# mayabechlerspeicher/Graph-Neural-Additive-Networks---GNAN

Hardware: AMD Instinct MI355X
Metric: edges aggregated/sec, TensorGNAN forward (higher is better)
Workload: dtype f32

## Files before the change

graph-neural-additive-networks---gnan_amd/_lib.py:

```python
from __future__ import annotations

import ctypes as C
import os
from typing import Optional

import torch

_HERE = os.path.dirname(os.path.abspath(__file__))
LIB_PATH = os.environ.get("GNAN_HIP_LIB") or os.path.join(_HERE, "libgnan_hip.so")
ABI_VERSION = 51
ERR_BAD_ARG, ERR_UNSUPPORTED, ERR_HIP, ERR_WORKSPACE = -1, -2, -3, -4

GNAN_F32, GNAN_BF16 = 0, 1
FMLP_AUTO, FMLP_LANE, FMLP_MFMA, FMLP_PWL = 0, 1, 2, 3
MAX_CODES = 256


class GnanHipError(RuntimeError):
    pass


class FmlpArgs(C.Structure):
    _fields_ = [
        ("x", C.c_void_p), ("n", C.c_int64), ("x_stride", C.c_int64),
# ... 130 lines not shown
        ("s_total", C.c_void_p), ("weight_by_col", C.c_int32), ("minus_rest", C.c_int32),
        ("reduce_cr", C.c_int32), ("scatter_out", C.c_int32), ("Y", C.c_void_p), ("y_stride", C.c_int64),
        ("long_threshold", C.c_int64), ("long_rows", C.c_void_p), ("long_slice_ptr", C.c_void_p),
        ("n_long", C.c_int32), ("n_slices", C.c_int32), ("slice_edges", C.c_int32),
        ("workspace", C.c_void_p), ("workspace_bytes", C.c_size_t),
        ("s_by_code", C.c_int32), ("nnz", C.c_int64), ("packed_index", C.c_int32),
        ("hot_lo", C.c_int64), ("hot_rows", C.c_int32), ("shell_out", C.c_void_p),
        ("cls_index", C.c_void_p), ("cls_slice_start", C.c_void_p), ("cls_slice_row", C.c_void_p), ("cls_slot_slice", C.c_void_p),
        ("cls_n_slots", C.c_int32),
        ("short_lmax", C.c_int32), ("short_row", C.c_void_p), ("short_pair", C.c_void_p),
        ("self_sum", C.c_void_p), ("self_parts", C.c_int32),
        ("seg_index", C.c_void_p), ("seg_start", C.c_void_p), ("seg_row", C.c_void_p), ("cls_seg_ptr", C.c_void_p),
        ("seg_mask", C.c_void_p), ("seg_q_lo", C.c_int64), ("seg_q_hi", C.c_int64), ("n_seg", C.c_int32),
        ("seg_max_per_class", C.c_int32),
        ("hub_index", C.c_void_p), ("hub_seg_start", C.c_void_p), ("hub_seg_row", C.c_void_p), ("hub_seg_slot", C.c_void_p),
        ("hub_row_slot_ptr", C.c_void_p), ("hub_cls_seg_ptr", C.c_void_p), ("hub_q_lo", C.c_int64), ("n_hub", C.c_int32),
        ("n_hub_seg", C.c_int32), ("hub_seg_max_per_class", C.c_int32),
        ("stream_index", C.c_void_p), ("stream_cls_pair_ptr", C.c_void_p), ("stream_cls_chunk_ptr", C.c_void_p),
        ("stream_chunk_first_seg", C.c_void_p), ("stream_seg_slot", C.c_void_p), ("stream_row_slot_ptr", C.c_void_p),
        ("stream_q_lo", C.c_int64), ("stream_q_hi", C.c_int64), ("stream_chunk", C.c_int32), ("stream_code", C.c_int32),
        ("n_stream_seg", C.c_int32), ("stream_max_chunks_per_class", C.c_int32),
        ("stream_row_seg", C.c_void_p),
        ("q_hub", C.c_int64),
    ]


SHORT_LMAX = 8
SPMM_KERNEL_NONE, SPMM_KERNEL_ROWS, SPMM_KERNEL_HOT = 0, 1, 2


class SpmmLaunchInfo(C.Structure):
    _fields_ = [
        ("vec", C.c_int32), ("lpr", C.c_int32), ("smalld", C.c_int32), ("dense", C.c_int32), ("kernel", C.c_int32),
        ("classed", C.c_int32), ("n_slice_blocks", C.c_int32), ("n_tile_blocks", C.c_int32), ("n_tiles", C.c_int32),
        ("row_q0", C.c_int64), ("short_tile", C.c_int32 * (SHORT_LMAX + 1)),
        ("n_seg_blocks", C.c_int32), ("n_segs", C.c_int32), ("n_hub_seg_blocks", C.c_int32), ("n_hub_segs", C.c_int32),
        ("n_stream_blocks", C.c_int32), ("n_stream_segs", C.c_int32),
    ]

    def as_dict(self) -> dict:
        d = {name: getattr(self, name) for name, _ in self._fields_}
        d["short_tile"] = list(self.short_tile)
        return d


class ClassedPlanArgs(C.Structure):
    _fields_ = [
        ("rowptr", C.c_void_p), ("rowptr_is64", C.c_int32), ("col", C.c_void_p), ("code", C.c_void_p), ("row_ids", C.c_void_p),
        ("long_rows", C.c_void_p), ("n_long", C.c_int32), ("slice_edges", C.c_int32),
        ("workspace", C.c_void_p), ("workspace_bytes", C.c_size_t), ("totals", C.c_void_p),
        ("index", C.c_void_p), ("slice_start", C.c_void_p), ("slice_row", C.c_void_p), ("slice_ptr", C.c_void_p),
        ("slot_slice", C.c_void_p), ("n_slots", C.c_int64),
    ]


class SortedCsrArgs(C.Structure):
    _fields_ = [
        ("n_rows", C.c_int64), ("nnz", C.c_int64), ("rowptr", C.c_void_p), ("rowptr_is64", C.c_int32), ("col", C.c_void_p),
        ("code", C.c_void_p), ("cnt", C.c_void_p), ("D", C.c_int32), ("pack_shift", C.c_int32), ("order", C.c_void_p),
        ("rowptr_s", C.c_void_p), ("col_s", C.c_void_p), ("code_s", C.c_void_p), ("colp_s", C.c_void_p), ("cnt_s", C.c_void_p),
        ("workspace", C.c_void_p), ("workspace_bytes", C.c_size_t),
    ]


class CsrTransposeArgs(C.Structure):
    _fields_ = [
# ... 561 lines not shown
```

graph-neural-additive-networks---gnan_amd/aggregate.py:

```python
from __future__ import annotations

import functools
from dataclasses import dataclass
from typing import NamedTuple, Optional

import torch

from . import _lib
from . import functional as Fn
from .functional import StackedMLP
from .graph import LONG_ROW_THRESHOLD, HopGraph

DENSE_SLICE_MAX_ROWS = 16384
DENSE_SLICE_MIN_COLS = 512
WEIGHT_TABLE_MAX_BYTES = 1 << 30
NARROW_DS_MAX_WIDTH = 32


def _spmm_args(g: HopGraph, S, lut, use_cnt, s_total, out, row_ids, per_row_lut, weight_by_col=False,
               minus_rest=False, plan=None, workspace=None, reduce_cr=0, scatter_out=False,
               s_by_code=False, packed=False, hot_rows=0) -> _lib.SpmmArgs:
    D, Cw = lut.shape[-2], lut.shape[-1]
    packed = bool(packed and PACKED_INDEX and g.colp is not None and D <= 4 and Cw == 1 and not weight_by_col
                  and not minus_rest and not s_by_code)
# ... 24 lines not shown


def _hot_head_in_lds(g: HopGraph, head: int) -> bool:
    return g.hot_head_share(head) >= HOT_LDS_MIN_SHARE


FUSABLE_READOUT = (1, 2, 4)
DEGREE_SCHEDULE_MIN_WIDTH = 8
DEGREE_SORTED_COPY_MIN_ROWS = 1 << 16
WIDE_INDEX_LOADS = True
PACKED_INDEX = True
NARROW_SORTED_MIN_NNZ = 1 << 23
NARROW_SORTED_WALK = True
HOT_COLUMN_ROWS = True
HOT_ROWS_IN_LDS = True
HOT_LDS_FLOATS = 16384
HOT_LDS_MIN_SHARE = 0.25
DEGREE_SORTED_COPY = True
XCD_CLASSED_HUBS = True
CLASSED_MIN_ROW_BYTES = 128
CLASSED_MIN_NNZ = 1 << 24
SHORT_ROW_TILES = True
SHORT_ROW_LMAX = 4
CLASSED_ROWS = True
CLASSED_ROWS_MIN_NNZ = 1 << 24
CLASSED_ROWS_MIN_PAIRS = 33
BLOCKED_HUBS = True
BLOCKED_HUBS_MIN_NNZ = 1 << 24
BLOCKED_HUB_BLOCK_BYTES = 4 << 20
BLOCKED_HUB_BLOCKS = 4
BLOCKED_HUB_SEG_PAIRS = 256
PAIR_STREAM = True
PAIR_STREAM_MIN_NNZ = 1 << 24
PAIR_STREAM_MIN_PAIRS = 5
PAIR_STREAM_BLOCKS = 2
PAIR_STREAM_CHUNK_PAIRS = 32
HUB_STREAM = True
HUB_STREAM_MIN_NNZ = 1 << 24
HUB_STREAM_BLOCKS = 4
HUB_STREAM_CHUNK_PAIRS = 32
PAIR_STREAM_COMBINE_ROWS = 256
PAIR_STREAM_COMBINE_CAP = 4096


def append_hot_rows(S: torch.Tensor, hot: torch.Tensor, group: int = 1, room: Optional[torch.Tensor] = None) -> torch.Tensor:
    W = S.shape[1]
# ... 84 lines not shown
    else:
        by_col_table = per_row and weight_by_col and not use_cnt
        g, row_ids, plan, scatter = _wide_walk(g, row_ids, S.shape[1], by_col_table or (not per_row and not weight_by_col))
        short = scatter == 2 and SHORT_ROW_TILES and not per_row and not weight_by_col
    if (XCD_CLASSED_HUBS and plan is not None and not g.is_dense and S.shape[1] * S.element_size() >= CLASSED_MIN_ROW_BYTES
            and g.nnz >= CLASSED_MIN_NNZ and not weight_by_col and not minus_rest and not s_by_code and not g._cnt_by_col
            and n_hot == 0):
        classed = g.classed_hub_plan(row_ids if scatter != 2 else None)
        if classed is not None:
            plan = classed
    if from_counts:
        lut = lut_of_counts(g.cnt).detach().float().contiguous()
        per_row = True
    a = _spmm_args(g, S, lut, use_cnt, s_total, out, row_ids, per_row, weight_by_col, minus_rest, plan,
                   reduce_cr=reduce_cr, scatter_out=scatter, s_by_code=s_by_code, packed=True, hot_rows=n_hot)
    if short and a.packed_index:
        runs = g.short_row_runs(SHORT_ROW_LMAX)
        a.short_lmax, a.short_row, a.short_pair = runs.lmax, runs.row_ptr, runs.pair_ptr
    if self_sum is not None:
        _lib.require_device(self_sum)
        if self_sum.dtype != torch.float32 or self_sum.dim() != 2 or self_sum.shape[1] != n_out or not self_sum.is_contiguous():
            raise ValueError("self_sum must be a contiguous float32 [parts, n_rows] tensor")
        a.self_sum, a.self_parts = _lib.ptr(self_sum), int(self_sum.shape[0])
        if (scatter == 2 and a.packed_index and a.short_lmax > 0 and reduce_cr == 1 and s_total is not None
                and S.dtype == torch.float32 and (plan is None or plan.threshold == LONG_ROW_THRESHOLD)):
            W, lo, rows, hubs, both = S.shape[1], SHORT_ROW_LMAX + 1, None, None, None
            block_rows = max(1, BLOCKED_HUB_BLOCK_BYTES // (W * 4)) if W else 0
            if (HUB_STREAM and PAIR_STREAM and HUB_STREAM_CHUNK_PAIRS == PAIR_STREAM_CHUNK_PAIRS and g.nnz >= HUB_STREAM_MIN_NNZ
                    and 32 < W <= 256 and plan is not None and plan.n_long > 0):
                both = g.pair_stream_plan(max(PAIR_STREAM_MIN_PAIRS, lo), block_rows, PAIR_STREAM_BLOCKS, HUB_STREAM_CHUNK_PAIRS, None,
                                          HUB_STREAM_BLOCKS)
            if both is not None:
                both.bind(a)
            else:
                if PAIR_STREAM and g.nnz >= PAIR_STREAM_MIN_NNZ and 32 < W <= 256:
                    rows = g.pair_stream_plan(max(PAIR_STREAM_MIN_PAIRS, lo), block_rows, PAIR_STREAM_BLOCKS, PAIR_STREAM_CHUNK_PAIRS)
                if rows is None and CLASSED_ROWS and g.nnz >= CLASSED_ROWS_MIN_NNZ:
                    rows = g.classed_row_plan(max(CLASSED_ROWS_MIN_PAIRS, lo))
                if BLOCKED_HUBS and g.nnz >= BLOCKED_HUBS_MIN_NNZ and plan is not None and plan.n_long > 0:
                    hubs = g.blocked_hub_plan(block_rows, BLOCKED_HUB_BLOCKS, BLOCKED_HUB_SEG_PAIRS)
                for wide in (rows, hubs):
                    if wide is not None:
                        wide.bind(a)
    need = _lib.lib().gnan_spmm_fwd_workspace_bytes(a)
    ws = None
    if need:
# ... 677 lines not shown
```

graph-neural-additive-networks---gnan_amd/csrc/spmm.hip:

```cpp
#include "spmm_common.hpp"

namespace {

template <int VEC>
__device__ __forceinline__ Vec<VEC> hot_gather(const Params& p, const float* hot, int c) {
  const int64_t r = static_cast<int64_t>(c) - p.hot_lo;
  const bool is_hot = r >= 0 && r < p.hot_n;
  const Vec<VEC> g = load_vec<VEC>(static_cast<const float*>(p.S) + (is_hot ? p.hot_lo : static_cast<int64_t>(c)) * VEC);
  const int rl = is_hot ? static_cast<int>(r) : 0;
  Vec<VEC> l;
  if constexpr (VEC == 4) {
    const float4 t = *reinterpret_cast<const float4*>(hot + rl * 4);
    l.v[0] = t.x; l.v[1] = t.y; l.v[2] = t.z; l.v[3] = t.w;
  } else if constexpr (VEC == 2) {
    const float2 t = *reinterpret_cast<const float2*>(hot + rl * 2);
    l.v[0] = t.x; l.v[1] = t.y;
  } else {
    l.v[0] = hot[rl];
  }
  Vec<VEC> out;
#pragma unroll
  for (int v = 0; v < VEC; ++v) out.v[v] = is_hot ? l.v[v] : g.v[v];
  return out;
}
// ... 396 lines not shown
  const bool dense = a->rowptr == nullptr;
  return vec == 4 ? launch_shell_lpr<4>(p, lpr, dense, st) : launch_shell_lpr<1>(p, lpr, dense, st);
}

extern "C" int gnan_spmm_fwd_describe(const gnan_spmm_args* a, gnan_spmm_launch_info* out) {
  GNAN_REQUIRE(out != nullptr, "spmm describe: null output");
  if (int rc = validate(a)) return rc;
  *out = gnan_spmm_launch_info{};
  if (a->n_rows == 0) return GNAN_OK;
  Route r;
  if (int rc = pick_route(a, &r)) return rc;
  out->vec = r.vec; out->lpr = r.lpr; out->smalld = r.smalld; out->dense = r.dense;
  out->kernel = r.hot ? GNAN_SPMM_KERNEL_HOT : GNAN_SPMM_KERNEL_ROWS;
  if (r.hot) return GNAN_OK;
  Params p = make_params(a);
  if (int rc = plan_tiles(p, r.vec, r.lpr, r.dense, r.smalld, a->seg_max_per_class, a->hub_seg_max_per_class)) return rc;
  out->n_seg_blocks = p.n_seg_blocks; out->n_segs = p.n_seg_blocks > 0 ? a->n_seg : 0;
  out->n_hub_seg_blocks = p.n_hub_blocks; out->n_hub_segs = p.n_hub_blocks > 0 ? a->n_hub_seg : 0;
  out->n_stream_blocks = gnan::stream_blocks(a, r.lpr); out->n_stream_segs = out->n_stream_blocks > 0 ? a->n_stream_seg : 0;
  out->classed = p.cls_index != nullptr;
  out->n_slice_blocks = p.n_slice_blocks; out->n_tile_blocks = p.n_tile_blocks; out->n_tiles = p.n_tiles;
  out->row_q0 = p.row_q0;
  for (int L = 0; L <= GNAN_SHORT_LMAX; ++L) out->short_tile[L] = p.short_tile[L];
  return GNAN_OK;
}

extern "C" int gnan_spmm_fwd(const gnan_spmm_args* a, gnan_stream_t stream) {
  if (int rc = validate(a)) return rc;
  if (a->n_rows == 0) return GNAN_OK;
  const size_t need = gnan_spmm_fwd_workspace_bytes(a);
  if (need > 0 && (a->workspace == nullptr || a->workspace_bytes < need))
    return gnan::fail(GNAN_ERR_WORKSPACE, "spmm: workspace %zu B < required %zu B", a->workspace_bytes, need);
  const Params p = make_params(a);
  Route r;
  if (int rc = pick_route(a, &r)) return rc;
  hipStream_t st = static_cast<hipStream_t>(stream);
  if (r.hot) return a->W == 1 ? launch_hot<1>(p, st) : (a->W == 2 ? launch_hot<2>(p, st) : launch_hot<4>(p, st));
  if (int rc0 = gnan::launch_stream(a, r.lpr, st)) return rc0;
  const int rc = r.vec == 8 ? gnan::launch_lpr<8>(a, r.lpr, r.dense, r.smalld, st)
                            : (r.vec == 4 ? gnan::launch_lpr<4>(a, r.lpr, r.dense, r.smalld, st) : gnan::launch_lpr<1>(a, r.lpr, r.dense, r.smalld, st));
  if (rc) return rc;
  if (int rc2 = launch_fixup(p, st)) return rc2;
  if (int rc2 = launch_hub_combine(p, st)) return rc2;
  if (int rc2 = launch_seg_combine(p, st)) return rc2;
  return gnan::launch_stream_combine(a, st);
}
```

graph-neural-additive-networks---gnan_amd/csrc/spmm_common.hpp:

```cpp
#pragma once
#include "common.hpp"

#include <cstdlib>
#include <type_traits>

namespace {

using gnan::kWave;

struct Params {
  int64_t n_rows, n_cols;
  int64_t nnz;
  const void* rowptr;
  int rowptr_is64;
  const int32_t* col;
  const uint8_t* code;
  const int32_t* row_ids;
  const void* S;
  int W;
  int64_t s_stride;
  const float* lut;
  int64_t lut_row_stride;
  int D, Cw;
  const int32_t* cnt;
// ... 24 lines not shown
  int n_tile_blocks, n_tiles;
  int64_t row_q0;
  int64_t short_row[GNAN_SHORT_LMAX + 2], short_pair[GNAN_SHORT_LMAX + 1];
  int short_tile[GNAN_SHORT_LMAX + 1];
  const float* self_sum;
  int self_parts;
  const int32_t* seg_index;
  const int64_t* seg_start;
  const int32_t* seg_row;
  const int32_t* cls_seg_ptr;
  const uint8_t* seg_mask;
  float* seg_partial;
  int64_t seg_q_lo, seg_q_hi;
  int n_seg_blocks;
  const int32_t* hub_index;
  const int64_t* hub_seg_start;
  const int32_t* hub_seg_row;
  const int32_t* hub_seg_slot;
  const int32_t* hub_row_slot_ptr;
  const int32_t* hub_cls_seg_ptr;
  float* hub_partial;
  int64_t hub_q_lo;
  int n_hub, n_hub_blocks;
};

__device__ __forceinline__ int64_t load_rowptr(const Params& p, int64_t i) {
  return p.rowptr_is64 ? static_cast<const int64_t*>(p.rowptr)[i]
                       : static_cast<int64_t>(static_cast<const int32_t*>(p.rowptr)[i]);
}

__device__ __forceinline__ int64_t adj_row(const Params& p, int64_t q) {
  return (p.row_ids && p.scatter_out != 2) ? static_cast<int64_t>(p.row_ids[q]) : q;
}
__device__ __forceinline__ int64_t out_row(const Params& p, int64_t q, int64_t i) {
  return p.scatter_out == 2 ? static_cast<int64_t>(p.row_ids[q]) : (p.scatter_out ? i : q);
}

__device__ __forceinline__ float self_term(const Params& p, int64_t o) {
  float a = p.self_sum[o];
  for (int k = 1; k < p.self_parts; ++k) a += p.self_sum[k * p.n_rows + o];
  return a;
}

template <int VEC>
struct Vec {
  float v[VEC];
// ... 163 lines not shown
}

template <int N>
__device__ __forceinline__ void load_index_run(const int32_t* col, const uint8_t* code, int (&colv)[N], int (&codev)[N]) {
  static_assert(N == 4 || N == 8 || N == 16, "whole dwords of codes");
  load_col_run<N>(col, colv);
  unsigned cw[4] = {0u, 0u, 0u, 0u};
  if constexpr (N == 16) {
    const uint4_a1 v = *reinterpret_cast<const uint4_a1*>(code);
    cw[0] = v.x; cw[1] = v.y; cw[2] = v.z; cw[3] = v.w;
  } else if constexpr (N == 8) {
    const uint2_a1 v = *reinterpret_cast<const uint2_a1*>(code);
    cw[0] = v.x; cw[1] = v.y;
  } else {
    cw[0] = *reinterpret_cast<const uint1_a1*>(code);
  }
#pragma unroll
  for (int r = 0; r < N; ++r) codev[r] = static_cast<int>((cw[r / 4] >> (8 * (r % 4))) & 0xffu);
}

template <int CTRL>
__device__ __forceinline__ float dpp_row(float v) {
  return __int_as_float(__builtin_amdgcn_update_dpp(0, __float_as_int(v), CTRL, 0xf, 0xf, false));
}

__host__ __device__ constexpr int short_rows_per_group(int L) { return L == 0 ? 8 : (8 / L > 0 ? 8 / L : 1); }

__host__ __device__ constexpr bool short_tiles_serve(int vec, int lpr, bool smalld, bool packed, bool bycode) {
  return vec == 4 && lpr >= 16 && smalld && packed && !bycode;
}

__device__ __forceinline__ int slice_owner(const Params& p, int s) {
  int a = 0, b = p.n_long;
  while (b - a > 1) {
    const int mid = (a + b) >> 1;
    if (p.long_slice_ptr[mid] <= s) a = mid; else b = mid;
  }
  return a;
}
__device__ __forceinline__ int slice_owner_from(const Params& p, int a, int s) {
  while (p.long_slice_ptr[a + 1] <= s) ++a;
  return a;
}
template <bool DENSE = false>
__device__ __forceinline__ void slice_range(const Params& p, int64_t i, int a, int s, int64_t& lo, int64_t& hi) {
  const int64_t row_lo = DENSE ? 0 : load_rowptr(p, i), row_hi = DENSE ? p.n_cols : load_rowptr(p, i + 1);
// ... 22 lines not shown
  if (a->s_dtype != GNAN_F32 && a->s_dtype != GNAN_BF16) return gnan::fail(GNAN_ERR_BAD_ARG, "spmm: unknown operand dtype %d", a->s_dtype);
  if (a->s_dtype == GNAN_BF16) {
    if (a->W % 8 != 0 || a->s_stride % 8 != 0 || reinterpret_cast<uintptr_t>(a->S) % 16 != 0 || a->rowptr == nullptr)
      return gnan::fail(GNAN_ERR_UNSUPPORTED, "spmm: bf16 operand rows need the CSR layout, W %% 8 == 0 and 16-B aligned rows");
    if (a->reduce_cr == 0 && (a->y_stride % 4 != 0 || reinterpret_cast<uintptr_t>(a->Y) % 16 != 0))
      return gnan::fail(GNAN_ERR_UNSUPPORTED, "spmm: bf16 operand rows need a 16-B aligned fp32 output");
    if (a->s_total && reinterpret_cast<uintptr_t>(a->s_total) % 16 != 0)
      return gnan::fail(GNAN_ERR_UNSUPPORTED, "spmm: s_total must be 16-B aligned");
  }
  GNAN_REQUIRE(!(a->weight_by_col && a->s_total), "spmm: weight_by_col excludes the rest-bucket term (add it outside)");
  GNAN_REQUIRE(!a->s_by_code || (a->rowptr != nullptr && a->s_total == nullptr && a->s_dtype == GNAN_F32),
               "spmm: s_by_code needs the CSR layout, fp32 rows and no rest-bucket term");
  if (a->s_by_code && a->W > 32)
    return gnan::fail(GNAN_ERR_UNSUPPORTED, "spmm: s_by_code covers operand rows of at most 32 columns (got W=%d)", a->W);
  GNAN_REQUIRE(!a->scatter_out || a->row_ids, "spmm: scatter_out needs row_ids");
  if (a->packed_index && (a->rowptr == nullptr || a->D > 4 || a->Cw != 1 || a->weight_by_col || a->minus_rest || a->s_by_code ||
                          a->n_cols > static_cast<int64_t>(kPackMask) + 1))
    return gnan::fail(GNAN_ERR_UNSUPPORTED, "spmm: packed index entries need the CSR layout, D <= 4, one weight channel, plain "
                      "forward weights and n_cols <= 2^29");
  if (a->self_sum && !(a->packed_index && a->scatter_out == 2 && a->s_dtype == GNAN_F32 && a->reduce_cr == 1 && a->lut_row_stride == 0 &&
                       a->self_parts >= 1 && a->hot_rows == 0 && a->shell_out == nullptr))
    return gnan::fail(GNAN_ERR_UNSUPPORTED, "spmm: self_sum is served over a packed degree-sorted copy (scatter_out 2) with a global "
                      "small-D table, fp32 rows and reduce_cr == 1 (self_parts >= 1)");
  if (a->reduce_cr != 0) {
    const int cr = a->reduce_cr;
    if (!(cr == 1 || cr == 2 || cr == 4) || a->W % cr != 0)
      return gnan::fail(GNAN_ERR_UNSUPPORTED, "spmm: fused read-out needs reduce_cr in {1, 2, 4} dividing W (got %d, W=%d)",
                        cr, a->W);
    GNAN_REQUIRE(a->y_stride >= cr, "spmm: y_stride smaller than reduce_cr");
  }
  if (a->short_lmax != 0) {
    const int lm = a->short_lmax;
    GNAN_REQUIRE(lm > 0 && lm <= GNAN_SHORT_LMAX, "spmm: short_lmax must be in [0, %d] (got %d)", GNAN_SHORT_LMAX, lm);
    GNAN_REQUIRE(a->short_row && a->short_pair, "spmm: short_lmax > 0 needs the short_row / short_pair host arrays");
    GNAN_REQUIRE(a->rowptr != nullptr && a->scatter_out == 2 && a->short_row[0] == 0 && a->short_row[lm + 1] <= a->n_rows,
                 "spmm: short-row runs need a degree-sorted copy (CSR, scatter_out 2) and runs from row 0 within n_rows");
    for (int L = 0; L <= lm; ++L) {
      const int64_t n = a->short_row[L + 1] - a->short_row[L];
      const int64_t end = a->short_pair[L] + n * L;
      GNAN_REQUIRE(n >= 0 && a->short_pair[L] >= 0 && (a->nnz <= 0 || end <= a->nnz) && (L == lm || end == a->short_pair[L + 1]),
                   "spmm: short-row run %d is inconsistent (rows %lld, first pair %lld)", L, static_cast<long long>(n),
                   static_cast<long long>(a->short_pair[L]));
    }
  }
  if (a->seg_index) {
    if (!self_route_with_tiles(a))
// ... 93 lines not shown
  p.seg_index = a->seg_index; p.seg_start = a->seg_start; p.seg_row = a->seg_row; p.cls_seg_ptr = a->cls_seg_ptr;
  p.seg_mask = a->seg_mask;
  p.seg_q_lo = p.seg_q_hi = 0;
  p.n_seg_blocks = 0;
  p.seg_partial = nullptr;
  if (a->seg_index) {
    p.seg_q_lo = a->seg_q_lo; p.seg_q_hi = a->seg_q_hi;
    p.seg_partial = static_cast<float*>(a->workspace) + seg_partial_offset(a);
  } else if (a->stream_index) {
    p.seg_q_lo = a->stream_q_lo; p.seg_q_hi = a->stream_q_hi;
  }
  p.hub_index = a->hub_index; p.hub_seg_start = a->hub_seg_start; p.hub_seg_row = a->hub_seg_row; p.hub_seg_slot = a->hub_seg_slot;
  p.hub_row_slot_ptr = a->hub_row_slot_ptr; p.hub_cls_seg_ptr = a->hub_cls_seg_ptr;
  p.hub_partial = nullptr;
  p.hub_q_lo = a->n_rows;
  p.n_hub = p.n_hub_blocks = 0;
  if (a->hub_index) {
    p.hub_q_lo = a->hub_q_lo; p.n_hub = a->n_hub;
    p.hub_partial = static_cast<float*>(a->workspace) + hub_partial_offset(a);
    p.long_threshold = a->long_threshold;
  }
  p.n_tile_blocks = p.n_tiles = 0;
  p.row_q0 = 0;
  for (int L = 0; L <= GNAN_SHORT_LMAX + 1; ++L) p.short_row[L] = L <= p.short_lmax + 1 && runs ? a->short_row[L] : 0;
  for (int L = 0; L <= GNAN_SHORT_LMAX; ++L) {
    p.short_pair[L] = L <= p.short_lmax && runs ? a->short_pair[L] : 0;
    p.short_tile[L] = 0;
  }
  return p;
}

inline void pick_tiling(const gnan_spmm_args* a, const float* out, int64_t out_stride, int* vec, int* lpr) {
  *vec = 1;
  if (a->W % 4 == 0 && a->s_stride % 4 == 0 && out_stride % 4 == 0 && aligned(a->S, 16) && aligned(out, 16) &&
      (!a->s_total || aligned(a->s_total, 16)))
    *vec = 4;
  *lpr = 1;
  while (*lpr * *vec < a->W && *lpr < kWave) *lpr <<= 1;
}

inline int plan_tiles(Params& p, int vec, int lpr, bool dense, bool smalld, int seg_max = 0, int hub_seg_max = 0) {
  const int G = kWave / lpr;
  if (short_tiles_serve(vec, lpr, smalld, p.packed, p.s_by_code) && p.short_lmax > 0 && !dense && p.scatter_out == 2 &&
      lpr * vec >= p.W && p.nnz > 0) {
    int64_t t = 0;
    for (int L = 0; L <= p.short_lmax; ++L) {
      p.short_tile[L] = static_cast<int>(t);
      const int64_t per = static_cast<int64_t>(G) * short_rows_per_group(L);
      t += (p.short_row[L + 1] - p.short_row[L] + per - 1) / per;
    }
    if (t > 0x7fffffffLL - 3) return gnan::fail(GNAN_ERR_UNSUPPORTED, "spmm: too many short-row tiles for one launch");
    p.n_tiles = static_cast<int>(t);
    p.n_tile_blocks = static_cast<int>((t + 3) / 4);
    p.row_q0 = p.short_row[p.short_lmax + 1];
  } else {
    p.short_lmax = 0;
  }
  if (p.seg_index) {
    if (!(p.short_lmax > 0 && p.self_sum && p.seg_q_lo >= p.row_q0))
      return gnan::fail(GNAN_ERR_UNSUPPORTED, "spmm: classed row segments need the tiled self_sum variant (fp32 rows of 16 lanes or more)");
    const int64_t per = 4 * static_cast<int64_t>(G);
    const int64_t nb = 8 * ((static_cast<int64_t>(seg_max) + per - 1) / per);
    if (nb > 0x3fffffffLL) return gnan::fail(GNAN_ERR_UNSUPPORTED, "spmm: too many row segments for one launch");
    p.n_seg_blocks = static_cast<int>(nb);
  }
  if (p.hub_index) {
    if (!(p.short_lmax > 0 && p.self_sum && p.hub_q_lo >= p.row_q0))
      return gnan::fail(GNAN_ERR_UNSUPPORTED, "spmm: blocked hub segments need the tiled self_sum variant (fp32 rows of 16 lanes or more)");
    const int64_t per = 4 * static_cast<int64_t>(G);
    const int64_t nb = 8 * ((static_cast<int64_t>(hub_seg_max) + per - 1) / per);
    if (nb > 0x3fffffffLL) return gnan::fail(GNAN_ERR_UNSUPPORTED, "spmm: too many hub segments for one launch");
    p.n_hub_blocks = static_cast<int>(nb);
  }
  return GNAN_OK;
}


template <class F>
int dispatch_lpr(int lpr, F&& f) {
  switch (lpr) {
    case 1: return f(std::integral_constant<int, 1>{});
    case 2: return f(std::integral_constant<int, 2>{});
    case 4: return f(std::integral_constant<int, 4>{});
    case 8: return f(std::integral_constant<int, 8>{});
    case 16: return f(std::integral_constant<int, 16>{});
    case 32: return f(std::integral_constant<int, 32>{});
    default: return f(std::integral_constant<int, 64>{});
  }
}

inline size_t slice_T_bytes(const gnan_spmm_args* a) {
  const size_t bytes = a->n_long > 0 ? static_cast<size_t>(a->n_slices) * 4 * static_cast<size_t>(a->W) * sizeof(float) : 0;
  return (bytes + 15) / 16 * 16;
}

inline int forward_only_self_sum(const gnan_spmm_args* a, const char* who) {
  GNAN_REQUIRE(a->self_sum == nullptr, "%s: self_sum is read by gnan_spmm_fwd only", who);
  return GNAN_OK;
}
inline int forward_only_index(const gnan_spmm_args* a, const char* who, bool reads_packed = false) {
  GNAN_REQUIRE(a->cls_index == nullptr, "%s: the classed hub plan is read by gnan_spmm_fwd only", who);
  GNAN_REQUIRE(a->hub_index == nullptr, "%s: blocked hub segments are read by gnan_spmm_fwd only", who);
  GNAN_REQUIRE(a->stream_index == nullptr, "%s: the pair stream is read by gnan_spmm_fwd only", who);
  GNAN_REQUIRE(reads_packed || !a->packed_index, "%s: packed index entries are read by gnan_spmm_fwd only", who);
  return GNAN_OK;
}

using gnan::cu_count;
}

namespace gnan {
template <int VEC>
int launch_lpr(const gnan_spmm_args* a, int lpr, bool dense, bool smalld, hipStream_t st);
int stream_blocks(const gnan_spmm_args* a, int lpr);
int launch_stream(const gnan_spmm_args* a, int lpr, hipStream_t st);
int launch_stream_combine(const gnan_spmm_args* a, hipStream_t st);
}
```

graph-neural-additive-networks---gnan_amd/csrc/spmm_fwd_body.hpp:

```cpp
#pragma once
#include "spmm_common.hpp"

namespace {

template <int VEC, int LPR, bool DENSE, bool SMALLD, bool BYCODE, bool PACKED = false, bool SELF = false>
__device__ __forceinline__ void rows_body(const Params& p, const int64_t block_id) {
  constexpr int G = kWave / LPR;
  constexpr int TILE = LPR * VEC;
  constexpr int UNROLL = VEC == 8 ? 2 : 4;
  constexpr int IW = LPR >= 8 ? LPR : 16;
  constexpr int IPL = IW / LPR;
  const int lane = threadIdx.x & (kWave - 1);
  const int wave = threadIdx.x / kWave;
  const int sub = lane % LPR;
  const int slot = lane / LPR;
  int64_t q = p.row_q0 + (block_id * (blockDim.x / kWave) + wave) * G + slot;
  if constexpr (SELF) {
    if (q >= p.seg_q_lo) q += p.seg_q_hi - p.seg_q_lo;
  }
  if (q >= p.n_rows) return;
  const int64_t i = adj_row(p, q);
  int64_t lo, hi, code_base;
  if constexpr (DENSE) {
    lo = 0;
// ... 191 lines not shown
    float v = 0.f;
    if (r < nr && d < p.D) {
      v = p.lut[(qg + r) * p.lut_row_stride + d];
      if (p.cnt) {
        const int c = p.cnt[(qg + r) * p.cnt_stride + d];
        v = v / static_cast<float>(c > 1 ? c : 1);
      }
    }
    const float wr = __shfl(v, (sub & ~3) + rest, LPR);
    wrv[k] = 0.f;
    if (p.s_total) {
      wrv[k] = wr;
      v = d < rest ? v - wr : 0.f;
    }
    wv[k] = v;
  }
  Raw<VEC> s[NP > 0 ? NP : 1];
#pragma unroll
  for (int j = 0; j < NP; ++j) {
    const unsigned en = static_cast<unsigned>(__shfl(static_cast<int>(ent), j, LPR));
    s[j].zero();
    if (j < nr * L && col_ok) s[j].load(p.S, static_cast<int64_t>(en & kPackMask), p.s_stride, cw);
  }
#pragma unroll
  for (int r = 0; r < R; ++r) {
    if (r >= nr) break;
    Vec<VEC> acc;
#pragma unroll
    for (int v = 0; v < VEC; ++v) acc.v[v] = 0.f;
#pragma unroll
    for (int l = 0; l < L; ++l) {
      int d = static_cast<int>(static_cast<unsigned>(__shfl(static_cast<int>(ent), r * L + l, LPR)) >> kPackShift);
      d = d < rest ? d : rest;
      const float w = __shfl(wv[4 * r / LPR], (4 * r) % LPR + d, LPR);
      const Vec<VEC> sv = s[r * L + l].widen();
#pragma unroll
      for (int v = 0; v < VEC; ++v) acc.v[v] = fmaf(w, sv.v[v], acc.v[v]);
    }
    const float w_rest = __shfl(wrv[4 * r / LPR], (4 * r) % LPR, LPR);
    const int64_t o = __shfl(orow, r, LPR);
    float red[4] = {0.f, 0.f, 0.f, 0.f};
    if (col_ok) {
      if (p.s_total) {
        const Vec<VEC> tot = load_vec<VEC>(p.s_total + cw);
#pragma unroll
        for (int v = 0; v < VEC; ++v) acc.v[v] = fmaf(w_rest, tot.v[v], acc.v[v]);
      }
      if (p.reduce_cr == 0) {
        store_vec<VEC>(p.Y + o * p.y_stride + cw, acc);
      } else {
#pragma unroll
        for (int v = 0; v < VEC; ++v) {
          const int ch = (cw + v) & (p.reduce_cr - 1);
#pragma unroll
          for (int c = 0; c < 4; ++c) red[c] += ch == c ? acc.v[v] : 0.f;
        }
      }
    }
    if (p.reduce_cr) {
#pragma unroll
      for (int off = 1; off < LPR; off <<= 1) {
#pragma unroll
        for (int c = 0; c < 4; ++c) red[c] += __shfl_xor(red[c], off);
      }
      float w_self = 0.f;
      if constexpr (SELF) w_self = __shfl(wv[4 * r / LPR], (4 * r) % LPR, LPR);
      if (sub == 0) {
        if constexpr (SELF) red[0] = fmaf(w_self, self_term(p, o), red[0]);
        for (int c = 0; c < p.reduce_cr; ++c) p.Y[o * p.y_stride + c] = red[c];
      }
    }
  }
}

template <int VEC, int LPR, bool SELF>
__device__ __forceinline__ void short_tiles(const Params& p, int t) {
  if (t >= p.n_tiles) return;
  int L = 0;
  int64_t k = t, q0 = 0, q1 = p.short_row[1], e0 = p.short_pair[0];
#pragma unroll
  for (int l = 1; l <= GNAN_SHORT_LMAX; ++l) {
    if (l <= p.short_lmax && t >= p.short_tile[l]) {
      L = l; k = t - p.short_tile[l]; q0 = p.short_row[l]; q1 = p.short_row[l + 1]; e0 = p.short_pair[l];
    }
  }
  constexpr int G = kWave / LPR;
  const int slot = (threadIdx.x & (kWave - 1)) / LPR;
#define GNAN_SHORT_CASE(LL)                                                                       \
  case LL: {                                                                                      \
    constexpr int R = short_rows_per_group(LL);                                              \
    const int64_t qg = q0 + (k * G + slot) * R;                                                   \
    short_tile<VEC, LPR, LL, SELF>(p, qg, q1, e0 + (qg - q0) * LL);                                     \
// ... 49 lines not shown
      Vec<VEC> sv[FLY];
#pragma unroll
      for (int u = 0; u < FLY; ++u) {
        const int j = j0 + u < m ? j0 + u : m - 1;
        const unsigned en = static_cast<unsigned>(__shfl(ent, j, LPR));
        sv[u] = load_vec<VEC>(Sl + static_cast<int64_t>(en & kPackMask) * p.s_stride);
      }
#pragma unroll
      for (int u = 0; u < FLY; ++u) {
        const bool ok = j0 + u < m;
        const int j = ok ? j0 + u : m - 1;
        int d = static_cast<int>(static_cast<unsigned>(__shfl(ent, j, LPR)) >> kPackShift);
        d = d < rest ? d : rest;
        const float w = ok ? sw.pick(d) : 0.f;
#pragma unroll
        for (int v = 0; v < VEC; ++v) acc.v[v] = ok ? fmaf(w, sv[u].v[v], acc.v[v]) : acc.v[v];
      }
    }
  }
  float r = 0.f;
#pragma unroll
  for (int v = 0; v < VEC; ++v) r += acc.v[v];
  r = col_ok ? r : 0.f;
  r += dpp_row<0xB1>(r);
  r += dpp_row<0x4E>(r);
  r += dpp_row<0x141>(r);
  r += dpp_row<0x140>(r);
#pragma unroll
  for (int off = 16; off < LPR; off <<= 1) r += __shfl_xor(r, off);
  if constexpr (HUB) {
    if (sub == 0) p.hub_partial[p.hub_seg_slot[s]] = r;
  } else {
    if (sub == 0) p.seg_partial[(q - p.seg_q_lo) * 8 + cls] = r;
  }
}

template <int VEC, int LPR, bool SMALLD, bool DENSE, bool BYCODE, bool PACKED = false>
__device__ __forceinline__ void slice_body(const Params& p, const int blk) {
  constexpr int G = kWave / LPR;
  constexpr int TILE = LPR * VEC;
  constexpr int NW = 4;
  __shared__ float red[NW][2][TILE];
  const int lane = threadIdx.x & (kWave - 1);
  const int wave = threadIdx.x / kWave;
  const int sub = lane % LPR;
  const int slot = lane / LPR;
  const bool classed = !DENSE && p.cls_index != nullptr;
  int s = blk, a = 0;
  int64_t lo, hi;
  if (classed) {
    const int e = ((blk >> 3) * NW + wave) * 8 + (blk & 7);
    s = e < p.cls_n_slots ? p.cls_slot_slice[e] : -1;
// ... 127 lines not shown
    }
    if constexpr (short_tiles_serve(VEC, LPR, SMALLD, PACKED, BYCODE)) {
      if (static_cast<int>(blockIdx.x) < front + p.n_tile_blocks) {
        short_tiles<VEC, LPR, SELF>(p, (static_cast<int>(blockIdx.x) - front) * (blockDim.x / kWave) + threadIdx.x / kWave);
        return;
      }
    }
    rows_body<VEC, LPR, false, SMALLD, BYCODE, PACKED, SELF>(p, static_cast<int64_t>(blockIdx.x) - front - p.n_tile_blocks);
  } else {
    if (p.n_slices > 0) {
      slice_body<VEC, LPR, SMALLD, true, false>(p, static_cast<int>(blockIdx.x));
      return;
    }
    rows_body<VEC, LPR, true, SMALLD, false>(p, static_cast<int64_t>(blockIdx.x));
  }
}

template <int VEC, int LPR>
int launch(const gnan_spmm_args* a, bool dense, bool smalld, hipStream_t st) {
  constexpr int G = kWave / LPR;
  const int rows_per_block = 4 * G;
  Params p = make_params(a);
  if (int rc = plan_tiles(p, VEC, LPR, dense, smalld, a->seg_max_per_class, a->hub_seg_max_per_class)) return rc;
  const int n_slices = p.n_slices;
  const int64_t walked = p.hub_q_lo - p.row_q0 - (p.seg_q_hi - p.seg_q_lo);
  const int64_t blocks = dense && n_slices > 0
                             ? n_slices
                             : (walked + rows_per_block - 1) / rows_per_block + p.n_slice_blocks + p.n_hub_blocks + p.n_seg_blocks +
                                   p.n_tile_blocks;
  if (blocks > 0x7fffffffLL) return gnan::fail(GNAN_ERR_UNSUPPORTED, "spmm: too many rows for one launch");
  if (blocks == 0) return GNAN_OK;
  const dim3 grid(static_cast<unsigned>(blocks)), block(256);
  if (p.s_by_code) {
    if constexpr (VEC <= 4 && VEC * LPR <= 32) {
      if (smalld) {
        hipLaunchKernelGGL((spmm_kernel<VEC, LPR, false, true, true>), grid, block, 0, st, p);
      } else {
        hipLaunchKernelGGL((spmm_kernel<VEC, LPR, false, false, true>), grid, block, 0, st, p);
      }
    } else {
      return gnan::fail(GNAN_ERR_UNSUPPORTED, "spmm: s_by_code covers operand rows of at most 32 columns");
    }
  } else if (dense) {
    if constexpr (VEC != 8) {
      hipLaunchKernelGGL((spmm_kernel<VEC, LPR, true, false>), grid, block, 0, st, p);
    } else {
// ... 27 lines not shown
```

graph-neural-additive-networks---gnan_amd/csrc/spmm_stream.hip:

```cpp
#include "spmm_common.hpp"

namespace {

struct StreamParams {
  const float* S;
  int W;
  int64_t s_stride;
  const int32_t* index;
  const int32_t* cls_pair_ptr;
  const int32_t* cls_chunk_ptr;
  const int32_t* chunk_first_seg;
  const int32_t* row_seg;
  const int32_t* row_slot_ptr;
  float* partial;
  int64_t q_lo;
  int n_rows;
  int n_seg;
  int chunk;
  int code;
};

constexpr unsigned kStreamLast = 1u << 31;

template <int LPR>
__device__ __forceinline__ float group_sum(float r) {
  r += dpp_row<0xB1>(r);
  r += dpp_row<0x4E>(r);
  r += dpp_row<0x141>(r);
  r += dpp_row<0x140>(r);
#pragma unroll
  for (int off = 16; off < LPR; off <<= 1) r += __shfl_xor(r, off);
  return r;
}

template <int LPR>
__global__ __launch_bounds__(256) __attribute__((amdgpu_waves_per_eu(8)))
void spmm_stream_kernel(const StreamParams p) {
  static_assert(LPR >= 16, "a DPP row per lane group, one index entry per lane and round");
  constexpr int VEC = 4;
  constexpr int G = kWave / LPR;
  constexpr int IW = 16;
  constexpr int FLY = 4;
  const int lane = threadIdx.x & (kWave - 1);
  const int wave = threadIdx.x / kWave;
  const int sub = lane % LPR;
  const int slot = lane / LPR;
  const int cls = static_cast<int>(blockIdx.x) & 7;
  const int t0 = p.cls_chunk_ptr[cls];
  const int g = ((static_cast<int>(blockIdx.x) >> 3) * 4 + wave) * G + slot;
  if (g >= p.cls_chunk_ptr[cls + 1] - t0) return;
  const int64_t lo = p.cls_pair_ptr[cls] + static_cast<int64_t>(g) * p.chunk;
  const int64_t left = p.cls_pair_ptr[cls + 1] - lo;
  const int n = static_cast<int>(left < p.chunk ? left : p.chunk);
  const int32_t* idx = p.index + lo;
  const int seg0 = p.chunk_first_seg[t0 + g];
  const bool col_ok = sub * VEC < p.W;
// ... 173 lines not shown
```

include/gnan_hip.h:

```cpp
#ifndef GNAN_HIP_H
#define GNAN_HIP_H

#include <stddef.h>
#include <stdint.h>

#ifdef __cplusplus
extern "C" {
#endif
#pragma GCC visibility push(default)

#define GNAN_ABI_VERSION 51

typedef void* gnan_stream_t;

enum gnan_status {
  GNAN_OK = 0,
  GNAN_ERR_BAD_ARG = -1,
  GNAN_ERR_UNSUPPORTED = -2,
  GNAN_ERR_HIP = -3,
  GNAN_ERR_WORKSPACE = -4
};

enum gnan_dtype { GNAN_F32 = 0, GNAN_BF16 = 1 };

// ... 364 lines not shown
  const int32_t* hub_index;
  const int64_t* hub_seg_start;
  const int32_t* hub_seg_row;
  const int32_t* hub_seg_slot;
  const int32_t* hub_row_slot_ptr;
  const int32_t* hub_cls_seg_ptr;
  int64_t hub_q_lo;
  int32_t n_hub;
  int32_t n_hub_seg;
  int32_t hub_seg_max_per_class;
  const int32_t* stream_index;
  const int32_t* stream_cls_pair_ptr;
  const int32_t* stream_cls_chunk_ptr;
  const int32_t* stream_chunk_first_seg;
  const int32_t* stream_seg_slot;
  const int32_t* stream_row_slot_ptr;
  int64_t stream_q_lo, stream_q_hi;
  int32_t stream_chunk;
  int32_t stream_code;
  int32_t n_stream_seg;
  int32_t stream_max_chunks_per_class;
  const int32_t* stream_row_seg;
  int64_t q_hub;
} gnan_spmm_args;

size_t gnan_spmm_fwd_workspace_bytes(const gnan_spmm_args* a);
int gnan_spmm_fwd(const gnan_spmm_args* a, gnan_stream_t stream);

#define GNAN_SPMM_KERNEL_NONE 0
#define GNAN_SPMM_KERNEL_ROWS 1
#define GNAN_SPMM_KERNEL_HOT 2
typedef struct gnan_spmm_launch_info {
  int32_t vec;
  int32_t lpr;
  int32_t smalld;
  int32_t dense;
  int32_t kernel;
  int32_t classed;
  int32_t n_slice_blocks;
  int32_t n_tile_blocks;
  int32_t n_tiles;
  int64_t row_q0;
  int32_t short_tile[GNAN_SHORT_LMAX + 1];
  int32_t n_seg_blocks;
  int32_t n_segs;
  int32_t n_hub_seg_blocks;
  int32_t n_hub_segs;
  int32_t n_stream_blocks;
  int32_t n_stream_segs;
} gnan_spmm_launch_info;

int gnan_spmm_fwd_describe(const gnan_spmm_args* a, gnan_spmm_launch_info* out);

typedef struct gnan_sorted_csr_args {
  int64_t n_rows;
  int64_t nnz;
  const void* rowptr;
  int32_t rowptr_is64;
  const int32_t* col;
  const uint8_t* code;
  const int32_t* cnt;
  int32_t D;
  int32_t pack_shift;
  int32_t* order;
  void* rowptr_s;
  int32_t* col_s;
  uint8_t* code_s;
  int32_t* colp_s;
  int32_t* cnt_s;
  void* workspace;
  size_t workspace_bytes;
} gnan_sorted_csr_args;
// ... 845 lines not shown
```

Before: 30.91 billion.

## Serve pairless short rows with a thread-per-row lone kernel outside the tile walk

Rows with no pairs (length-0 short rows) in the degree-sorted self_sum route are removed from the tiled wave-per-row kernel and handled by a new kernel that uses one thread per row. It reads s_total once into LDS and computes the w_rest-weighted total plus the self term directly. The tiled SELF path is also reworked: s_total and the self term are loaded once ahead of the row loop, and a DPP group_sum replaces the generic reduce_cr shuffle. This adds a kernel launch and ABI fields, and changes the summation order for the lone rows.

```diff
diff --git a/graph-neural-additive-networks---gnan_amd/_lib.py b/graph-neural-additive-networks---gnan_amd/_lib.py
--- a/graph-neural-additive-networks---gnan_amd/_lib.py
+++ b/graph-neural-additive-networks---gnan_amd/_lib.py
@@ -176,6 +176,7 @@
         ("n_stream_seg", C.c_int32), ("stream_max_chunks_per_class", C.c_int32),
         ("stream_row_seg", C.c_void_p),
         ("q_hub", C.c_int64),
+        ("lone_rows", C.c_int32),
     ]
 
 
@@ -190,12 +191,20 @@
         ("row_q0", C.c_int64), ("short_tile", C.c_int32 * (SHORT_LMAX + 1)),
         ("n_seg_blocks", C.c_int32), ("n_segs", C.c_int32), ("n_hub_seg_blocks", C.c_int32), ("n_hub_segs", C.c_int32),
         ("n_stream_blocks", C.c_int32), ("n_stream_segs", C.c_int32),
-    ]
-
-    def as_dict(self) -> dict:
-        d = {name: getattr(self, name) for name, _ in self._fields_}
+        ("n_lone_rows", C.c_int64), ("n_lone_blocks", C.c_int32), ("n_tile_blocks_skipped", C.c_int32),
+    ]
+
+    LONE_FIELDS = ("n_lone_rows", "n_lone_blocks", "n_tile_blocks_skipped")
+
+    def as_dict(self) -> "LaunchPartition":
+        d = LaunchPartition({name: getattr(self, name) for name, _ in self._fields_ if name not in self.LONE_FIELDS})
         d["short_tile"] = list(self.short_tile)
+        d.lone = {name: getattr(self, name) for name in self.LONE_FIELDS}
         return d
+
+
+class LaunchPartition(dict):
+    lone: dict = {}
 
 
 class ClassedPlanArgs(C.Structure):
diff --git a/graph-neural-additive-networks---gnan_amd/aggregate.py b/graph-neural-additive-networks---gnan_amd/aggregate.py
--- a/graph-neural-additive-networks---gnan_amd/aggregate.py
+++ b/graph-neural-additive-networks---gnan_amd/aggregate.py
@@ -70,6 +70,7 @@
 CLASSED_MIN_NNZ = 1 << 24
 SHORT_ROW_TILES = True
 SHORT_ROW_LMAX = 4
+LONE_ROWS = True
 CLASSED_ROWS = True
 CLASSED_ROWS_MIN_NNZ = 1 << 24
 CLASSED_ROWS_MIN_PAIRS = 33
@@ -200,6 +201,7 @@
         if self_sum.dtype != torch.float32 or self_sum.dim() != 2 or self_sum.shape[1] != n_out or not self_sum.is_contiguous():
             raise ValueError("self_sum must be a contiguous float32 [parts, n_rows] tensor")
         a.self_sum, a.self_parts = _lib.ptr(self_sum), int(self_sum.shape[0])
+        a.lone_rows = int(LONE_ROWS and a.short_lmax > 0)
         if (scatter == 2 and a.packed_index and a.short_lmax > 0 and reduce_cr == 1 and s_total is not None
                 and S.dtype == torch.float32 and (plan is None or plan.threshold == LONG_ROW_THRESHOLD)):
             W, lo, rows, hubs, both = S.shape[1], SHORT_ROW_LMAX + 1, None, None, None
diff --git a/graph-neural-additive-networks---gnan_amd/csrc/spmm.hip b/graph-neural-additive-networks---gnan_amd/csrc/spmm.hip
--- a/graph-neural-additive-networks---gnan_amd/csrc/spmm.hip
+++ b/graph-neural-additive-networks---gnan_amd/csrc/spmm.hip
@@ -442,6 +442,7 @@
   out->n_slice_blocks = p.n_slice_blocks; out->n_tile_blocks = p.n_tile_blocks; out->n_tiles = p.n_tiles;
   out->row_q0 = p.row_q0;
   for (int L = 0; L <= GNAN_SHORT_LMAX; ++L) out->short_tile[L] = p.short_tile[L];
+  out->n_lone_rows = p.lone_n; out->n_lone_blocks = gnan::lone_blocks(p.lone_n); out->n_tile_blocks_skipped = p.n_tile_blocks - lone_tile_blocks(p);
   return GNAN_OK;
 }
 
@@ -460,6 +461,9 @@
   const int rc = r.vec == 8 ? gnan::launch_lpr<8>(a, r.lpr, r.dense, r.smalld, st)
                             : (r.vec == 4 ? gnan::launch_lpr<4>(a, r.lpr, r.dense, r.smalld, st) : gnan::launch_lpr<1>(a, r.lpr, r.dense, r.smalld, st));
   if (rc) return rc;
+  if (r.vec == 4 && r.smalld) {
+    if (int rc2 = gnan::launch_lone(a, r.lpr, st)) return rc2;
+  }
   if (int rc2 = launch_fixup(p, st)) return rc2;
   if (int rc2 = launch_hub_combine(p, st)) return rc2;
   if (int rc2 = launch_seg_combine(p, st)) return rc2;
diff --git a/graph-neural-additive-networks---gnan_amd/csrc/spmm_common.hpp b/graph-neural-additive-networks---gnan_amd/csrc/spmm_common.hpp
--- a/graph-neural-additive-networks---gnan_amd/csrc/spmm_common.hpp
+++ b/graph-neural-additive-networks---gnan_amd/csrc/spmm_common.hpp
@@ -70,6 +70,9 @@
   float* hub_partial;
   int64_t hub_q_lo;
   int n_hub, n_hub_blocks;
+  int lone;
+  int64_t lone_n;
+  int tile_lo;
 };
 
 __device__ __forceinline__ int64_t load_rowptr(const Params& p, int64_t i) {
@@ -279,6 +282,18 @@
 template <int CTRL>
 __device__ __forceinline__ float dpp_row(float v) {
   return __int_as_float(__builtin_amdgcn_update_dpp(0, __float_as_int(v), CTRL, 0xf, 0xf, false));
+}
+
+template <int LPR>
+__device__ __forceinline__ float group_sum(float r) {
+  static_assert(LPR >= 16, "whole DPP rows");
+  r += dpp_row<0xB1>(r);
+  r += dpp_row<0x4E>(r);
+  r += dpp_row<0x141>(r);
+  r += dpp_row<0x140>(r);
+#pragma unroll
+  for (int off = 16; off < LPR; off <<= 1) r += __shfl_xor(r, off);
+  return r;
 }
 
 __host__ __device__ constexpr int short_rows_per_group(int L) { return L == 0 ? 8 : (8 / L > 0 ? 8 / L : 1); }
@@ -347,6 +362,7 @@
                        a->self_parts >= 1 && a->hot_rows == 0 && a->shell_out == nullptr))
     return gnan::fail(GNAN_ERR_UNSUPPORTED, "spmm: self_sum is served over a packed degree-sorted copy (scatter_out 2) with a global "
                       "small-D table, fp32 rows and reduce_cr == 1 (self_parts >= 1)");
+  GNAN_REQUIRE(!a->lone_rows || a->self_sum, "spmm: lone_rows (the rows without a pair, a thread each) is served on the self_sum route only");
   if (a->reduce_cr != 0) {
     const int cr = a->reduce_cr;
     if (!(cr == 1 || cr == 2 || cr == 4) || a->W % cr != 0)
@@ -486,6 +502,9 @@
   }
   p.n_tile_blocks = p.n_tiles = 0;
   p.row_q0 = 0;
+  p.lone = a->lone_rows != 0 && a->self_sum != nullptr;
+  p.lone_n = 0;
+  p.tile_lo = 0;
   for (int L = 0; L <= GNAN_SHORT_LMAX + 1; ++L) p.short_row[L] = L <= p.short_lmax + 1 && runs ? a->short_row[L] : 0;
   for (int L = 0; L <= GNAN_SHORT_LMAX; ++L) {
     p.short_pair[L] = L <= p.short_lmax && runs ? a->short_pair[L] : 0;
@@ -517,6 +536,10 @@
     p.n_tiles = static_cast<int>(t);
     p.n_tile_blocks = static_cast<int>((t + 3) / 4);
     p.row_q0 = p.short_row[p.short_lmax + 1];
+    if (p.lone && p.self_sum && p.short_row[1] > p.short_row[0]) {
+      p.lone_n = p.short_row[1] - p.short_row[0];
+      p.tile_lo = p.short_tile[1];
+    }
   } else {
     p.short_lmax = 0;
   }
@@ -539,6 +562,15 @@
   return GNAN_OK;
 }
 
+
+inline int lone_tile_blocks(const Params& p) { return p.tile_lo > 0 ? (p.n_tiles - p.tile_lo + 3) / 4 : p.n_tile_blocks; }
+inline void leave_lone_tiles(Params& p) {
+  if (p.tile_lo <= 0) return;
+  p.n_tile_blocks = lone_tile_blocks(p);
+  p.n_tiles -= p.tile_lo;
+  for (int L = 1; L <= p.short_lmax; ++L) p.short_tile[L] -= p.tile_lo;
+  p.tile_lo = 0;
+}
 
 template <class F>
 int dispatch_lpr(int lpr, F&& f) {
@@ -579,4 +611,6 @@
 int stream_blocks(const gnan_spmm_args* a, int lpr);
 int launch_stream(const gnan_spmm_args* a, int lpr, hipStream_t st);
 int launch_stream_combine(const gnan_spmm_args* a, hipStream_t st);
-}
+int launch_lone(const gnan_spmm_args* a, int lpr, hipStream_t st);
+int lone_blocks(int64_t lone_n);
+}
diff --git a/graph-neural-additive-networks---gnan_amd/csrc/spmm_fwd_body.hpp b/graph-neural-additive-networks---gnan_amd/csrc/spmm_fwd_body.hpp
--- a/graph-neural-additive-networks---gnan_amd/csrc/spmm_fwd_body.hpp
+++ b/graph-neural-additive-networks---gnan_amd/csrc/spmm_fwd_body.hpp
@@ -237,6 +237,17 @@
     s[j].zero();
     if (j < nr * L && col_ok) s[j].load(p.S, static_cast<int64_t>(en & kPackMask), p.s_stride, cw);
   }
+  constexpr bool kSelfAhead = SELF && L != 1;
+  Vec<VEC> tot_all;
+  float a_self = 0.f;
+#pragma unroll
+  for (int v = 0; v < VEC; ++v) tot_all.v[v] = 0.f;
+  if constexpr (SELF) {
+    if (col_ok && p.s_total) tot_all = load_vec<VEC>(p.s_total + cw);
+  }
+  if constexpr (kSelfAhead) {
+    if (sub < nr) a_self = self_term(p, orow);
+  }
 #pragma unroll
   for (int r = 0; r < R; ++r) {
     if (r >= nr) break;
@@ -254,35 +265,52 @@
     }
     const float w_rest = __shfl(wrv[4 * r / LPR], (4 * r) % LPR, LPR);
     const int64_t o = __shfl(orow, r, LPR);
-    float red[4] = {0.f, 0.f, 0.f, 0.f};
-    if (col_ok) {
-      if (p.s_total) {
-        const Vec<VEC> tot = load_vec<VEC>(p.s_total + cw);
-#pragma unroll
-        for (int v = 0; v < VEC; ++v) acc.v[v] = fmaf(w_rest, tot.v[v], acc.v[v]);
-      }
-      if (p.reduce_cr == 0) {
-        store_vec<VEC>(p.Y + o * p.y_stride + cw, acc);
+    if constexpr (SELF) {
+      float y = 0.f;
+      if (col_ok) {
+        if (p.s_total) {
+#pragma unroll
+          for (int v = 0; v < VEC; ++v) acc.v[v] = fmaf(w_rest, tot_all.v[v], acc.v[v]);
+        }
+#pragma unroll
+        for (int v = 0; v < VEC; ++v) y += acc.v[v];
+      }
+      y = group_sum<LPR>(y);
+      const float w_self = __shfl(wv[4 * r / LPR], (4 * r) % LPR, LPR);
+      if constexpr (kSelfAhead) {
+        const float a = __shfl(a_self, r, LPR);
+        if (sub == 0) p.Y[o * p.y_stride] = fmaf(w_self, a, y);
       } else {
-#pragma unroll
-        for (int v = 0; v < VEC; ++v) {
-          const int ch = (cw + v) & (p.reduce_cr - 1);
-#pragma unroll
-          for (int c = 0; c < 4; ++c) red[c] += ch == c ? acc.v[v] : 0.f;
-        }
-      }
-    }
-    if (p.reduce_cr) {
-#pragma unroll
-      for (int off = 1; off < LPR; off <<= 1) {
-#pragma unroll
-        for (int c = 0; c < 4; ++c) red[c] += __shfl_xor(red[c], off);
-      }
-      float w_self = 0.f;
-      if constexpr (SELF) w_self = __shfl(wv[4 * r / LPR], (4 * r) % LPR, LPR);
-      if (sub == 0) {
-        if constexpr (SELF) red[0] = fmaf(w_self, self_term(p, o), red[0]);
-        for (int c = 0; c < p.reduce_cr; ++c) p.Y[o * p.y_stride + c] = red[c];
+        if (sub == 0) p.Y[o * p.y_stride] = fmaf(w_self, self_term(p, o), y);
+      }
+    } else {
+      float red[4] = {0.f, 0.f, 0.f, 0.f};
+      if (col_ok) {
+        if (p.s_total) {
+          const Vec<VEC> tot = load_vec<VEC>(p.s_total + cw);
+#pragma unroll
+          for (int v = 0; v < VEC; ++v) acc.v[v] = fmaf(w_rest, tot.v[v], acc.v[v]);
+        }
+        if (p.reduce_cr == 0) {
+          store_vec<VEC>(p.Y + o * p.y_stride + cw, acc);
+        } else {
+#pragma unroll
+          for (int v = 0; v < VEC; ++v) {
+            const int ch = (cw + v) & (p.reduce_cr - 1);
+#pragma unroll
+            for (int c = 0; c < 4; ++c) red[c] += ch == c ? acc.v[v] : 0.f;
+          }
+        }
+      }
+      if (p.reduce_cr) {
+#pragma unroll
+        for (int off = 1; off < LPR; off <<= 1) {
+#pragma unroll
+          for (int c = 0; c < 4; ++c) red[c] += __shfl_xor(red[c], off);
+        }
+        if (sub == 0) {
+          for (int c = 0; c < p.reduce_cr; ++c) p.Y[o * p.y_stride + c] = red[c];
+        }
       }
     }
   }
@@ -378,12 +406,7 @@
 #pragma unroll
   for (int v = 0; v < VEC; ++v) r += acc.v[v];
   r = col_ok ? r : 0.f;
-  r += dpp_row<0xB1>(r);
-  r += dpp_row<0x4E>(r);
-  r += dpp_row<0x141>(r);
-  r += dpp_row<0x140>(r);
-#pragma unroll
-  for (int off = 16; off < LPR; off <<= 1) r += __shfl_xor(r, off);
+  r = group_sum<LPR>(r);
   if constexpr (HUB) {
     if (sub == 0) p.hub_partial[p.hub_seg_slot[s]] = r;
   } else {
@@ -557,6 +580,7 @@
   const int rows_per_block = 4 * G;
   Params p = make_params(a);
   if (int rc = plan_tiles(p, VEC, LPR, dense, smalld, a->seg_max_per_class, a->hub_seg_max_per_class)) return rc;
+  leave_lone_tiles(p);
   const int n_slices = p.n_slices;
   const int64_t walked = p.hub_q_lo - p.row_q0 - (p.seg_q_hi - p.seg_q_lo);
   const int64_t blocks = dense && n_slices > 0
diff --git a/graph-neural-additive-networks---gnan_amd/csrc/spmm_lone.hip b/graph-neural-additive-networks---gnan_amd/csrc/spmm_lone.hip
--- /dev/null
+++ b/graph-neural-additive-networks---gnan_amd/csrc/spmm_lone.hip
@@ -0,0 +1,60 @@
+#include "spmm_common.hpp"
+
+namespace {
+
+constexpr int kLoneBlock = 256;
+
+template <int N>
+__device__ __forceinline__ float lone_tree(const float* tot, const float w_rest, const int W, const int l0) {
+  if constexpr (N == 1) {
+    const float4 t = *reinterpret_cast<const float4*>(tot + 4 * l0);
+    float y = 0.f;
+    y += fmaf(w_rest, t.x, 0.f);
+    y += fmaf(w_rest, t.y, 0.f);
+    y += fmaf(w_rest, t.z, 0.f);
+    y += fmaf(w_rest, t.w, 0.f);
+    return 4 * l0 < W ? y : 0.f;
+  } else {
+    const float lo = lone_tree<N / 2>(tot, w_rest, W, l0);
+    const float hi = lone_tree<N / 2>(tot, w_rest, W, l0 + N / 2);
+    return lo + hi;
+  }
+}
+
+template <int LPR>
+__global__ __launch_bounds__(kLoneBlock) void spmm_lone_kernel(const Params p) {
+  __shared__ __attribute__((aligned(16))) float tot[LPR * 4];
+  for (int c = threadIdx.x; c < LPR * 4; c += kLoneBlock) tot[c] = (p.s_total != nullptr && c < p.W) ? p.s_total[c] : 0.f;
+  __syncthreads();
+  const int64_t q = p.short_row[0] + static_cast<int64_t>(blockIdx.x) * kLoneBlock + threadIdx.x;
+  if (q >= p.short_row[0] + p.lone_n) return;
+  const int64_t o = p.row_ids[q];
+  const int rest = p.D - 1;
+  const SmallW sw = small_weights(p, q);
+  float w_rest = 0.f, w_self = sw.w[0];
+  float y = 0.f;
+  if (p.s_total) {
+    w_rest = sw.pick(rest);
+    w_self = rest > 0 ? sw.w[0] - w_rest : 0.f;
+    y = lone_tree<LPR>(tot, w_rest, p.W, 0);
+  }
+  p.Y[o * p.y_stride] = fmaf(w_self, self_term(p, o), y);
+}
+
+}
+
+int gnan::launch_lone(const gnan_spmm_args* a, int lpr, hipStream_t st) {
+  if (!a->lone_rows) return GNAN_OK;
+  Params p = make_params(a);
+  if (int rc = plan_tiles(p, 4, lpr, false, true, a->seg_max_per_class, a->hub_seg_max_per_class)) return rc;
+  if (p.lone_n <= 0) return GNAN_OK;
+  const int64_t nb = (p.lone_n + kLoneBlock - 1) / kLoneBlock;
+  if (nb > 0x7fffffffLL) return gnan::fail(GNAN_ERR_UNSUPPORTED, "spmm: too many lone rows for one launch");
+  const dim3 grid(static_cast<unsigned>(nb)), block(kLoneBlock);
+  if (lpr == 16) hipLaunchKernelGGL(spmm_lone_kernel<16>, grid, block, 0, st, p);
+  else if (lpr == 32) hipLaunchKernelGGL(spmm_lone_kernel<32>, grid, block, 0, st, p);
+  else hipLaunchKernelGGL(spmm_lone_kernel<64>, grid, block, 0, st, p);
+  return gnan::check_launch("spmm_lone_kernel");
+}
+
+int gnan::lone_blocks(int64_t lone_n) { return static_cast<int>((lone_n + kLoneBlock - 1) / kLoneBlock); }
diff --git a/graph-neural-additive-networks---gnan_amd/csrc/spmm_stream.hip b/graph-neural-additive-networks---gnan_amd/csrc/spmm_stream.hip
--- a/graph-neural-additive-networks---gnan_amd/csrc/spmm_stream.hip
+++ b/graph-neural-additive-networks---gnan_amd/csrc/spmm_stream.hip
@@ -21,17 +21,6 @@
 };
 
 constexpr unsigned kStreamLast = 1u << 31;
-
-template <int LPR>
-__device__ __forceinline__ float group_sum(float r) {
-  r += dpp_row<0xB1>(r);
-  r += dpp_row<0x4E>(r);
-  r += dpp_row<0x141>(r);
-  r += dpp_row<0x140>(r);
-#pragma unroll
-  for (int off = 16; off < LPR; off <<= 1) r += __shfl_xor(r, off);
-  return r;
-}
 
 template <int LPR>
 __global__ __launch_bounds__(256) __attribute__((amdgpu_waves_per_eu(8)))
diff --git a/include/gnan_hip.h b/include/gnan_hip.h
--- a/include/gnan_hip.h
+++ b/include/gnan_hip.h
@@ -410,6 +410,7 @@
   int32_t stream_max_chunks_per_class;
   const int32_t* stream_row_seg;
   int64_t q_hub;
+  int32_t lone_rows;
 } gnan_spmm_args;
 
 size_t gnan_spmm_fwd_workspace_bytes(const gnan_spmm_args* a);
@@ -436,6 +437,9 @@
   int32_t n_hub_segs;
   int32_t n_stream_blocks;
   int32_t n_stream_segs;
+  int64_t n_lone_rows;
+  int32_t n_lone_blocks;
+  int32_t n_tile_blocks_skipped;
 } gnan_spmm_launch_info;
 
 int gnan_spmm_fwd_describe(const gnan_spmm_args* a, gnan_spmm_launch_info* out);
```

Result: faster. 34.41 billion, median of 6 (+11.3%).
